# ParCoreLab/aCG

Measured on AMD Instinct MI355X. Metric: CG iter/s (whole node), Queen_4147-shaped fp64, higher is better.
Workload: dtype fp64; 1 GPU; model=queen4147-like-27pt-dof3-G111, rows=4102893, solver=cg-classic, parallelism=slab1-rccl

## Files before the change

acg_amd/gen/device_slab.py:

```python

from __future__ import annotations

import numpy as np
import torch

from ..part.subdomain import HaloPattern
from .stencil import _blocks, _slab_bounds


class DeviceSlabSystem:

    def __init__(self, **kw):
        self.__dict__.update(kw)

    @property
    def nlocal(self):
        return self.nowned + self.nghost

    @property
    def nnzA(self):
        return self._nnzA

    @property
    def nnzO(self):
        return self._nnzO


def estimate_slab_gib(gx: int, gy: int, gz: int, spec: dict, rank: int,
                      nranks: int, matfree: bool = False) -> float:
    dof = spec["dof"]
# ... 189 lines not shown
        sendidx_parts.append(plane_rows(z1 - 1))
    sendcounts = [len(s) for s in sendidx_parts]
    sdispls = list(np.concatenate([[0], np.cumsum(sendcounts)[:-1]])) if sendcounts else []
    sendidx = (np.concatenate(sendidx_parts) if sendidx_parts
               else np.zeros(0, np.int64))
    halo = HaloPattern(
        senders=np.asarray(senders, dtype=np.int32),
        recvcounts=np.asarray(recvcounts, dtype=np.int64),
        rdispls=np.asarray(rdispls, dtype=np.int64),
        recipients=np.asarray(recipients, dtype=np.int32),
        sendcounts=np.asarray(sendcounts, dtype=np.int64),
        sdispls=np.asarray(sdispls, dtype=np.int64),
        sendidx=sendidx.astype(np.int32),
    )
    return DeviceSlabSystem(
        rank=rank, nparts=nranks, n_global=gx * gy * gz * dof,
        nowned=nowned, ninterior=ninterior_nodes * dof,
        nborder=nborder_nodes * dof, nghost=nghost,
        A_sell=(A_sellptr, A_cols, A_vals) if operator else None,
        A_bsell=A_bsell,
        O_sell=(O_sellptr, O_cols, O_vals) if operator else None,
        mf_tables=mf_tables,
        _nnzA=nnzA, _nnzO=nnzO, halo=halo, device=device,
    )
```

acg_amd/gen/stencil.py:

```python

from __future__ import annotations

import numpy as np

from ..core.symcsr import SymCSRMatrix
from ..part.subdomain import HaloPattern, LocalSystem

def _offsets_27():
    offs = [(dx, dy, dz, -1.0)
            for dz in (-1, 0, 1) for dy in (-1, 0, 1) for dx in (-1, 0, 1)
            if not (dx == 0 and dy == 0 and dz == 0)]
    return offs


STENCIL_5PT_2D = {
    "offsets": [(-1, 0, 0, -1.0), (1, 0, 0, -1.0), (0, -1, 0, -1.0), (0, 1, 0, -1.0)],
    "diag": 4.0,
    "dof": 1,
}
STENCIL_7PT_3D = {
    "offsets": [(-1, 0, 0, -1.0), (1, 0, 0, -1.0), (0, -1, 0, -1.0),
                (0, 1, 0, -1.0), (0, 0, -1, -1.0), (0, 0, 1, -1.0)],
    "diag": 6.0,
    "dof": 1,
# ... 55 lines not shown
            ii.append(gid * dof + a)
            jj.append(gid * dof + b)
            vv.append(np.full(nnodes, D[a, b]))
    for (dx, dy, dz, w) in spec["offsets"]:
        if (dz, dy, dx) <= (0, 0, 0):
            continue
        nx, ny, nz = X + dx, Y + dy, Z + dz
        ok = (nx >= 0) & (nx < gx) & (ny >= 0) & (ny < gy) & (nz >= 0) & (nz < gz)
        gi = gid[ok]
        gj = _node_id(nx[ok], ny[ok], nz[ok], gx, gy)
        for a in range(dof):
            for b in range(dof):
                if M[a, b] == 0.0:
                    continue
                ii.append(gi * dof + a)
                jj.append(gj * dof + b)
                vv.append(np.full(len(gi), w * M[a, b]))
    i = np.concatenate(ii)
    j = np.concatenate(jj)
    v = np.concatenate(vv)
    return SymCSRMatrix.from_coo(n, i, j, v)


def _slab_bounds(gz: int, rank: int, nranks: int) -> tuple[int, int]:
    z0 = (gz * rank) // nranks
    z1 = (gz * (rank + 1)) // nranks
    return z0, z1


def stencil_local_slab(gx: int, gy: int, gz: int, spec: dict,
                       rank: int, nranks: int) -> LocalSystem:
    dof = spec["dof"]
    z0, z1 = _slab_bounds(gz, rank, nranks)
    nz_own = z1 - z0
    if nz_own <= 0:
        raise ValueError(f"rank {rank} has no z-planes ({gz} planes / {nranks} ranks)")
    plane_nodes = gx * gy
    has_lo = rank > 0
    has_hi = rank < nranks - 1
    maxreach = max(abs(o[2]) for o in spec["offsets"])
    if maxreach > 1:
        raise ValueError("slab generator supports |dz| <= 1 stencils")
    border_planes = set()
    if has_lo:
        border_planes.add(z0)
    if has_hi:
# ... 122 lines not shown
        recipients.append(rank + 1)
        sendidx_parts.append(plane_rows(z1 - 1))
    if has_lo and has_hi:
        pass
    sendcounts = [len(s) for s in sendidx_parts]
    sdispls = list(np.concatenate([[0], np.cumsum(sendcounts)[:-1]])) if sendcounts else []
    sendidx = np.concatenate(sendidx_parts) if sendidx_parts else np.zeros(0, np.int64)

    halo = HaloPattern(
        senders=np.asarray(senders, dtype=np.int32),
        recvcounts=np.asarray(recvcounts, dtype=np.int64),
        rdispls=np.asarray(rdispls, dtype=np.int64),
        recipients=np.asarray(recipients, dtype=np.int32),
        sendcounts=np.asarray(sendcounts, dtype=np.int64),
        sdispls=np.asarray(sdispls, dtype=np.int64),
        sendidx=sendidx.astype(cdt),
    )
    return LocalSystem(
        rank=rank, nparts=nranks, n_global=gx * gy * gz * dof,
        nowned=nowned, ninterior=ninterior, nborder=nborder, nghost=nghost,
        A_rowptr=A_rowptr, A_colidx=A_cols.astype(cdt), A_vals=A_vals,
        O_rowptr=O_rowptr, O_colidx=O_cols.astype(cdt), O_vals=O_vals,
        owned_global=owned_global, ghost_global=ghost_global, halo=halo,
    )
```

acg_amd/ops/gpu_ops.py:

```python

from __future__ import annotations

import torch

try:
    from . import _acg_kernels as K
except ImportError as e:
    raise ImportError(
        "acg_amd HIP kernel extension (_acg_kernels) is not built. "
        "Run `python -m acg_amd.ops.build` (hipcc --offload-arch=gfx950). "
        f"Original error: {e}"
    ) from e

S_RR = K.S_RR
S_PT = K.S_PT
S_RR_PREV = K.S_RR_PREV
S_BNRM2 = K.S_BNRM2
S_GAMMA = K.S_GAMMA
S_DELTA = K.S_DELTA
S_GAMMA_PREV = K.S_GAMMA_PREV
S_ALPHA_PREV = K.S_ALPHA_PREV
S_NSLOTS = K.S_NSLOTS
MAXG = K.MAXG


def _stream() -> int:
    return torch.cuda.current_stream().cuda_stream


def alloc_scalars(device) -> torch.Tensor:
    return torch.zeros(S_NSLOTS, dtype=torch.float64, device=device)


def alloc_partials(device) -> torch.Tensor:
    return torch.zeros(2 * MAXG, dtype=torch.float64, device=device)


def pick_lanes(mean_nnz_per_row: float) -> int:
    if mean_nnz_per_row <= 4.0:
        return 4
    if mean_nnz_per_row <= 8.0:
        return 8
    if mean_nnz_per_row <= 16.0:
        return 16
    if mean_nnz_per_row <= 96.0:
        return 32
# ... 119 lines not shown
                1 if cols.dtype == torch.int64 else 0,
                vals.data_ptr(), x.data_ptr(), y.data_ptr(), accum,
                partials.data_ptr() if fuse else 0,
                scal.data_ptr() if fuse else 0, dotslot, dot_accum,
                variant, perm.data_ptr() if perm is not None else 0, val32,
                _stream())


def spmv_bsell(bptr: torch.Tensor, bcol: torch.Tensor, bvals: torch.Tensor,
               nnodes: int, dof: int, x: torch.Tensor, y: torch.Tensor, *,
               partials: torch.Tensor | None = None,
               scal: torch.Tensor | None = None, dotslot: int = -1,
               dot_accum: bool = True) -> None:
    val32 = _val32(bvals, "spmv_bsell")
    nslices = bptr.numel() - 1
    if nslices <= 0:
        return
    fuse = scal is not None and dotslot >= 0
    K.spmv_bsell(nslices, nnodes, dof, bptr.data_ptr(), bcol.data_ptr(),
                 bvals.data_ptr(), x.data_ptr(), y.data_ptr(),
                 partials.data_ptr() if fuse else 0,
                 scal.data_ptr() if fuse else 0, dotslot, dot_accum, val32,
                 _stream())


def stencil_spmv(mf, nrows_nodes: int, row0_node: int, x: torch.Tensor,
                 y: torch.Tensor, *, mato: bool = False,
                 partials: torch.Tensor | None = None,
                 scal: torch.Tensor | None = None, dotslot: int = -1,
                 dot_accum: bool = True) -> None:
    if nrows_nodes <= 0:
        return
    fuse = scal is not None and dotslot >= 0
    pp = partials.data_ptr() if fuse else 0
    sp = scal.data_ptr() if fuse else 0
    if not mato and mf["w7"] is not None:
        K.stencil_spmv7(mf["gx"] * mf["gy"], mf["gx"], mf["z0"], mf["z1"],
                        mf["gz"], mf["nown_nodes"], mf["pb"].data_ptr(),
                        mf["diag"], *mf["w7"], x.data_ptr(), y.data_ptr(),
                        pp, sp, dotslot, dot_accum, _stream())
        return
    K.stencil_spmv(nrows_nodes, row0_node, mf["gx"], mf["gy"], mf["gz"],
                   mf["nown_nodes"], mf["zs"].data_ptr(),
                   mf["pb"].data_ptr(), mf["offs"].data_ptr(), mf["ksten"],
                   mf["diag"], x.data_ptr(), y.data_ptr(), mato,
                   pp, sp, dotslot, dot_accum, _stream())
# ... 526 lines not shown
```

acg_amd/ops/kernels.hip:

```cpp
#define S_RR 0
#define S_PT 1
#define S_RR_PREV 2
#define S_BNRM2 3
#define S_GAMMA 4
#define S_DELTA 5
#define S_GAMMA_PREV 6
#define S_ALPHA_PREV 7
#define S_NSLOTS 8

#define BS_LD 8
#define BS_M 0
#define BS_XI 64
#define BS_XIC 128
#define BS_G 192
#define BS_ZETA 256
#define BS_ZINV 320
#define BS_C 384
#define BS_FLAG 448
#define BS_ITER 449
#define BS_SIZE 456
#define BLOCK_MAXG 2048
#define BLOCK_TAU 1e-6

#define MAXG 16384
// ... 185 lines not shown
        double acc[DOF];
        #pragma unroll
        for (int r = 0; r < DOF; ++r) acc[r] = 0.0;
        for (long j = 0; j < blen; ++j) {
            const int cb = ld_nt(c + j * WAVE);
            double xv[DOF];
            #pragma unroll
            for (int cc = 0; cc < DOF; ++cc) xv[cc] = x[(long)cb * DOF + cc];
            const ValT* __restrict__ vj = v + j * (DOF * DOF) * WAVE;
            #pragma unroll
            for (int k = 0; k < DOF * DOF; ++k) {
                const double a = (double)ld_nt(vj + bval_off<DOF * DOF>(k, lane));
                acc[k / DOF] += a * xv[k % DOF];
            }
        }
        const long node = s * WAVE + lane;
        if (node < nnodes) {
            #pragma unroll
            for (int r = 0; r < DOF; ++r) {
                y[node * DOF + r] = acc[r];
                if (FUSE_DOT) dacc += x[node * DOF + r] * acc[r];
            }
        }
    }
    if (FUSE_DOT) {
        dacc = block_reduce(dacc);
        if (threadIdx.x == 0) partials[blockIdx.x] = dacc;
    }
}

template <int DOF>
__global__ void __launch_bounds__(BLOCK)
k_spmv_bsell_daypx(long nslices, long nnodes,
                   const long* __restrict__ bptr,
                   const int* __restrict__ bcol,
                   const double* __restrict__ bvals,
                   const double* __restrict__ pold,
                   const double* __restrict__ rvec,
                   double* __restrict__ pnew,
                   double* __restrict__ y,
                   const double* __restrict__ scal,
                   double* __restrict__ partials) {
    const int lane = threadIdx.x & (WAVE - 1);
    const long wslice = ((long)blockIdx.x * BLOCK + threadIdx.x) >> 6;
    const long nw = ((long)gridDim.x * BLOCK) >> 6;
    const double beta = safe_div(scal[S_RR], scal[S_RR_PREV]);
// ... 692 lines not shown
                               (int)blocks, (double*)scal, dotslot, dot_accum ? 1 : 0);
            check_hip("spmv_bsell_reduce");
        }
        return;
    }
    #define LBS(D, FD) \
        hipLaunchKernelGGL((k_spmv_bsell<D, FD>), g, b, 0, (hipStream_t)stream, \
            nslices, nnodes, (const long*)bptr, (const int*)bcol, \
            (const double*)bvals, (const double*)x, (double*)y, (double*)partials)
    switch (dof) {
        case 2: if (fuse) { LBS(2, true); } else { LBS(2, false); } break;
        case 3: if (fuse) { LBS(3, true); } else { LBS(3, false); } break;
        case 4: if (fuse) { LBS(4, true); } else { LBS(4, false); } break;
        default: throw std::runtime_error("spmv_bsell: dof must be 2/3/4");
    }
    #undef LBS
    check_hip("spmv_bsell");
    if (fuse) {
        hipLaunchKernelGGL(k_reduce_partials, dim3(1), dim3(BLOCK), 0,
                           (hipStream_t)stream, (const double*)partials,
                           (int)blocks, (double*)scal, dotslot, dot_accum ? 1 : 0);
        check_hip("spmv_bsell_reduce");
    }
}

void spmv_bsell_daypx(long nslices, long nnodes, int dof, uintptr_t bptr,
                      uintptr_t bcol, uintptr_t bvals, uintptr_t pold,
                      uintptr_t rvec, uintptr_t pnew, uintptr_t y,
                      uintptr_t scal, uintptr_t partials, int dotslot,
                      uintptr_t stream) {
    if (nnodes == 0) return;
    long blocks = (nslices * WAVE + BLOCK - 1) / BLOCK;
    if (blocks > MAXG) blocks = MAXG;
    dim3 g((unsigned)blocks), b(BLOCK);
    #define LBD(D) \
        hipLaunchKernelGGL((k_spmv_bsell_daypx<D>), g, b, 0, (hipStream_t)stream, \
            nslices, nnodes, (const long*)bptr, (const int*)bcol, \
            (const double*)bvals, (const double*)pold, (const double*)rvec, \
            (double*)pnew, (double*)y, (const double*)scal, (double*)partials)
    switch (dof) {
        case 2: LBD(2); break;
        case 3: LBD(3); break;
        case 4: LBD(4); break;
        default: throw std::runtime_error("spmv_bsell_daypx: dof must be 2/3/4");
    }
    #undef LBD
// ... 1891 lines not shown
    m.def("spmv_sell", &spmv_sell);
    m.def("zero_scalars", &zero_scalars);
    m.def("cg_prep_pt", &cg_prep_pt);
    m.def("cg_prep_rr", &cg_prep_rr);
    m.def("dot", &dot);
    m.def("dot2", &dot2);
    m.def("axpy_ratio", &axpy_ratio);
    m.def("daypx_ratio", &daypx_ratio);
    m.def("cg_fused_update", &cg_fused_update);
    m.def("pcg_fused_update", &pcg_fused_update);
    m.def("bsell_diag_inv", &bsell_diag_inv);
    m.def("bjacobi_apply", &bjacobi_apply);
    m.def("bpcg_fused_update", &bpcg_fused_update);
    m.def("pipelined_fused", &pipelined_fused);
    m.def("sell_pipe", &sell_pipe);
    m.def("pipelined_finalize", &pipelined_finalize);
    m.def("pack_gather", &pack_gather);
    m.def("atomic_probe", &atomic_probe);
    m.def("cg_device", &cg_device);
    m.def("stencil_rowlen", &stencil_rowlen);
    m.def("stencil_fill", &stencil_fill);
    m.def("spmv_bsell", &spmv_bsell);
    m.def("spmv_bsell_daypx", &spmv_bsell_daypx);
    m.def("stencil_blocklen", &stencil_blocklen);
    m.def("stencil_bfill", &stencil_bfill);
    m.def("stencil_spmv", &stencil_spmv);
    m.def("stencil_pipe", &stencil_pipe);
    m.def("stencil_spmv7", &stencil_spmv7);
    m.def("stencil_pipe7", &stencil_pipe7);
    m.attr("S_RR") = S_RR;
    m.attr("S_PT") = S_PT;
    m.attr("S_RR_PREV") = S_RR_PREV;
    m.attr("S_BNRM2") = S_BNRM2;
    m.attr("S_GAMMA") = S_GAMMA;
    m.attr("S_DELTA") = S_DELTA;
    m.attr("S_GAMMA_PREV") = S_GAMMA_PREV;
    m.attr("S_ALPHA_PREV") = S_ALPHA_PREV;
    m.attr("S_NSLOTS") = S_NSLOTS;
    m.attr("MAXG") = MAXG;
}
```

acg_amd/ops/torch_ref.py:

```python

from __future__ import annotations

import math

import torch

S_RR, S_PT, S_RR_PREV, S_BNRM2 = 0, 1, 2, 3
S_GAMMA, S_DELTA, S_GAMMA_PREV, S_ALPHA_PREV = 4, 5, 6, 7
S_NSLOTS = 8
MAXG = 16384
OPERATOR_VALUE_DTYPES = (torch.float64, torch.float32)


def _vals64(vals, what: str):
    if vals.dtype not in OPERATOR_VALUE_DTYPES:
        raise TypeError(f"{what}: operator values must be float64 or "
                        f"float32, got {vals.dtype}")
    return vals.to(torch.float64)


def alloc_scalars(device="cpu") -> torch.Tensor:
    return torch.zeros(S_NSLOTS, dtype=torch.float64, device=device)


# ... 272 lines not shown
    if bptr.numel() - 1 <= 0:
        return
    n = nnodes * dof
    contrib = _bsell_contrib(bptr, bcol, bvals, nnodes, dof, x)
    y[:n] = contrib
    if scal is not None and dotslot >= 0:
        d = torch.dot(x[:n], contrib)
        scal[dotslot] = scal[dotslot] + d if dot_accum else d


def spmv_bsell_daypx(bptr, bcol, bvals, nnodes: int, dof: int, pold, rvec,
                     pnew, y, scal, partials, dotslot: int) -> None:
    if bptr.numel() - 1 <= 0:
        return
    n = nnodes * dof
    beta = _sdiv(float(scal[S_RR]), float(scal[S_RR_PREV]))
    pn = beta * pold[:n] + rvec[:n]
    contrib = _bsell_contrib(bptr, bcol, bvals, nnodes, dof, pn)
    pnew[:n] = pn
    y[:n] = contrib
    scal[dotslot] = torch.dot(pn, contrib)


def cg_prep_pt(scal) -> None:
    scal[S_PT] = 0.0


def cg_prep_rr(scal) -> None:
    scal[S_RR_PREV] = scal[S_RR].clone()


def dot(x, y, partials, scal, slot, n=None, accumulate=False) -> None:
    n = x.numel() if n is None else n
    d = torch.dot(x[:n], y[:n])
    scal[slot] = scal[slot] + d if accumulate else d


def dot2(r, w, partials, scal, n, accumulate=False) -> None:
    g = torch.dot(r[:n], r[:n])
    d = torch.dot(w[:n], r[:n])
    if accumulate:
        scal[S_GAMMA] += g
        scal[S_DELTA] += d
    else:
        scal[S_GAMMA] = g
        scal[S_DELTA] = d
# ... 616 lines not shown
```

acg_amd/part/subdomain.py:

```python

from __future__ import annotations

from dataclasses import dataclass, field

import numpy as np

from ..utils.errors import AcgError, ErrCode


@dataclass
class HaloPattern:

    senders: np.ndarray = field(default_factory=lambda: np.zeros(0, np.int32))
    recvcounts: np.ndarray = field(default_factory=lambda: np.zeros(0, np.int64))
    rdispls: np.ndarray = field(default_factory=lambda: np.zeros(0, np.int64))
    recipients: np.ndarray = field(default_factory=lambda: np.zeros(0, np.int32))
    sendcounts: np.ndarray = field(default_factory=lambda: np.zeros(0, np.int64))
    sdispls: np.ndarray = field(default_factory=lambda: np.zeros(0, np.int64))
    sendidx: np.ndarray = field(default_factory=lambda: np.zeros(0, np.int64))

    @property
    def nsenders(self) -> int:
        return len(self.senders)

# ... 9 lines not shown
    def recvsize(self) -> int:
        return int(self.recvcounts.sum()) if len(self.recvcounts) else 0


@dataclass
class LocalSystem:

    rank: int
    nparts: int
    n_global: int
    nowned: int
    ninterior: int
    nborder: int
    nghost: int
    A_rowptr: np.ndarray
    A_colidx: np.ndarray
    A_vals: np.ndarray
    O_rowptr: np.ndarray
    O_colidx: np.ndarray
    O_vals: np.ndarray
    owned_global: np.ndarray
    ghost_global: np.ndarray
    halo: HaloPattern

    @property
    def nlocal(self) -> int:
        return self.nowned + self.nghost

    @property
    def nnzA(self) -> int:
        return int(self.A_rowptr[-1])

    @property
    def nnzO(self) -> int:
        return int(self.O_rowptr[-1]) if len(self.O_rowptr) else 0

    def dump(self, file=None) -> None:
        import sys

        f = file or sys.stderr
        h = self.halo
        print(f"LocalSystem(rank={self.rank}/{self.nparts}, n_global={self.n_global})",
              file=f)
        print(f"  rows: owned={self.nowned} (interior={self.ninterior}, "
              f"border={self.nborder}), ghost={self.nghost}", file=f)
        print(f"  matA: nnz={self.nnzA}; matO: nnz={self.nnzO}", file=f)
# ... 148 lines not shown
```

acg_amd/solvers/hip.py:

```python

from __future__ import annotations

import math
import os
import sys
import time

import numpy as np
import torch

from ..dist.halo import HaloExchange
from ..ops import gpu_ops as ops
from ..part.subdomain import LocalSystem
from .base import (ColumnTolerances, SolveResult, block_results,
                   cg_flops_per_iter, check_multi_shapes, next_multi_k,
                   refine, solve_multi_by_column)


class LaggedReadback:

    def __init__(self, width: int, lag: int):
        self.lag = lag
        self._buf = [torch.zeros(width, dtype=torch.float64, pin_memory=True)
                     for _ in range(lag + 1)]
        self._ev = [torch.cuda.Event() for _ in range(lag + 1)]

    def push(self, k: int, src: torch.Tensor, stream) -> None:
        j = k % (self.lag + 1)
        if stream == torch.cuda.current_stream(stream.device):
            self._buf[j].copy_(src, non_blocking=True)
        else:
            with torch.cuda.stream(stream):
                self._buf[j].copy_(src, non_blocking=True)
        self._ev[j].record(stream)

    def event(self, k: int):
        return self._ev[k % (self.lag + 1)]

    def get(self, j: int) -> torch.Tensor:
# ... 11 lines not shown
                 profile: bool = False, matfree: bool = False,
                 force_format: str | None = None):
        self.local = local
        self.comm = comm
        if device is None:
            device = comm.device if comm is not None and comm.device is not None \
                else torch.device("cuda", 0)
        self.device = torch.device(device)
        L = local

        def up(a, dtype=None):
            t = torch.from_numpy(np.ascontiguousarray(a))
            return t.to(self.device, non_blocking=True)

        self.n = L.nowned
        self.nlocal = L.nowned + L.nghost
        self.sell = None
        self.sellO = None
        self.sell_perm = None
        self.A_rowptr = self.A_colidx = self.A_vals = None
        self.O_rowptr = self.O_colidx = self.O_vals = None
        self.lanesA = self.lanesO = lanes or 16
        self.bsell = None
        self.hybrid = None
        self.matfree = None
        if matfree:
            mf = getattr(L, "mf_tables", None)
            if mf is None:
                raise ValueError(
                    "matfree=True needs a device-generated dof=1 stencil "
                    "system (gen.device_slab with spec dof==1)")
            self.matfree = mf
        if hasattr(L, "A_sell"):
            self.sell = L.A_sell
            self.sellO = L.O_sell
            self.bsell = getattr(L, "A_bsell", None)
            if self.sell is None and self.matfree is None:
                raise ValueError("system generated with operator=False "
                                 "requires matfree=True")
        else:
            self.A_rowptr = up(L.A_rowptr)
            self.A_colidx = up(L.A_colidx)
            self.A_vals = up(L.A_vals)
            self.O_rowptr = up(L.O_rowptr)
            self.O_colidx = up(L.O_colidx)
            self.O_vals = up(L.O_vals)
            mean_nnz = L.nnzA / max(L.nowned, 1)
            self.lanesA = lanes or ops.pick_lanes(mean_nnz)
            mean_nnzO = L.nnzO / max(L.nborder, 1)
            self.lanesO = lanes or ops.pick_lanes(mean_nnzO)
            self._pick_format(L, up, use_sell, force_format)
        self.can_megafuse = (
            self.matfree is not None
            or (self.sell is not None and self.sell_perm is None
                and self.sell[1].dtype == torch.int32
                and (L.nnzO == 0 or (self.sellO is not None
                                     and self.sellO[1].dtype == torch.int32))))
        self.megafuse_auto = (self.can_megafuse
                              and (self.matfree is not None
                                   or L.nnzA / max(L.nowned, 1) <= 16.0))
        self.halo = HaloExchange(L.halo, L.nowned, self.device, comm)
        self.scal = ops.alloc_scalars(self.device)
        self.partials = ops.alloc_partials(self.device)
        from .profiling import EventProfiler

        self.prof = EventProfiler(profile)
        self.comm_stream = torch.cuda.Stream(self.device)
        self.allred_stream = torch.cuda.Stream(self.device)
        self.copy_stream = torch.cuda.Stream(self.device)
        self._rr_host = torch.zeros(1, dtype=torch.float64, pin_memory=True)
        self._ev_p = torch.cuda.Event()
        self._ev_recv = torch.cuda.Event()
        self._ev_rr = torch.cuda.Event()
        self.niterations_total = 0
        self._ws: dict = {}
        self._graphs: dict = {}
        self._nstag = 0
        self._vals32 = None
        self.multi_group = 8

    def _pick_format(self, L, up, use_sell: bool, force: str | None) -> None:
        from ..ops.torch_ref import bsell_from_csr, sell_from_csr

# ... 45 lines not shown
        def mk_bsell():
            for dof_try in (4, 3, 2):
                out = bsell_from_csr(L.A_rowptr, L.A_colidx, L.A_vals, dof_try)
                if out is None:
                    continue
                bptr_h, bcol_h, bvals_h, density = out
                if density >= 0.75:
                    self.bsell = (up(bptr_h), up(bcol_h), up(bvals_h), dof_try)
                    return True
            return False

        if force == "csr":
            return
        if force == "hybrid":
            mk_hybrid()
            return
        if force == "binned":
            mk_binned()
            return
        if force == "sell":
            mk_sell(1)
        elif force == "sigma":
            mk_sell(4096)
        elif force == "bsell":
            if not mk_bsell():
                raise ValueError("force_format=bsell: no dense dof x dof "
                                 "block structure (density < 0.75)")
        elif use_sell:
            waste = mk_sell(1)
            if waste > 0.3:
                self.sell = self.sellO = self.sell_perm = None
                waste = mk_sell(16)
                if waste > 0.5:
                    self.sell = self.sellO = self.sell_perm = None
                    mk_hybrid()
            mk_bsell()
        if self.sell is not None or self.bsell is not None:
            self.A_rowptr = self.A_colidx = self.A_vals = None

    def _workspace(self, key: str, names) -> dict:
        ws = self._ws.setdefault(key, {})
        for nm, nghost in names:
            if nm not in ws:
                n = self.nlocal if nghost else self.n
                off = 520 * self._nstag
                self._nstag += 1
                buf = torch.zeros(n + off, dtype=torch.float64,
                                  device=self.device)
                ws[nm] = buf[off:] if off else buf
        return ws


    def _allreduce_slot(self, slot: int, count: int = 1):
        if self.comm is not None and self.comm.size > 1:
            self.comm.allreduce_(self.scal[slot:slot + count])

    def _halo_fork(self, x: torch.Tensor, span=None) -> None:
        self._ev_p.record(torch.cuda.current_stream(self.device))
        self.comm_stream.wait_event(self._ev_p)
        if span is not None:
            span.__enter__()
# ... 40 lines not shown
        from .profiling import annotate_op_stats

        idxb = None
        if self.matfree is not None:
            idxb = -8.0
        elif self.bsell is not None:
            idxb = 4.0 / (self.bsell[3] ** 2)
        annotate_op_stats(res, self.local, self.prof.collect(),
                          idx_bytes_per_nnz=idxb)
        self.prof.reset()

    def _format_name(self) -> str:
        if self.matfree is not None:
            return "matrix-free"
        if hasattr(self.local, "A_sell"):
            return "device-generated"
        if self.bsell is not None:
            return "bsell"
        if self.sell is not None:
            return "sigma" if self.sell_perm is not None else "sell"
        if self.hybrid is not None:
            return "hybrid" if self.hybrid["sellptr"] is not None else "binned"
        return "csr"

    def _lowprec_values(self) -> torch.Tensor:
        if self._vals32 is None and self.n == 0:
            self._vals32 = torch.empty(0, dtype=torch.float32,
                                       device=self.device)
        if self._vals32 is None:
            fmt = self._format_name()
            if fmt not in ("sell", "sigma", "bsell"):
                raise ValueError(
                    f"the fp32-stored operator needs the SELL, sigma-SELL or "
                    f"BSELL format; this system uses {fmt}")
            src = self.bsell[2] if self.bsell is not None else self.sell[2]
            self._vals32 = src.to(torch.float32)
        return self._vals32

    def _spmv_overlapped(self, xfull: torch.Tensor, y: torch.Tensor,
                         fuse_dotslot: int = -1, lowprec: bool = False):
        L = self.local
        vals32 = self._lowprec_values() if lowprec else None
        have_halo = self.comm is not None and self.comm.size > 1
        if have_halo:
            halo_span = self.prof.span("halo", self.comm_stream)
            self._halo_fork(xfull, halo_span)
# ... 71 lines not shown

    def solve(self, b: torch.Tensor, x: torch.Tensor, maxits: int = 100,
              res_atol: float = 0.0, res_rtol: float = 1e-9,
              use_graph: bool | None = None,
              fold_daypx: bool | None = None,
              diff_atol: float = 0.0, diff_rtol: float = 0.0) -> SolveResult:
        return self._solve_classic(b, x, maxits, res_atol, res_rtol,
                                   use_graph, fold_daypx, diff_atol,
                                   diff_rtol, lowprec=False)

    def _solve_classic(self, b, x, maxits, res_atol, res_rtol,
                       use_graph=None, fold_daypx=None, diff_atol=0.0,
                       diff_rtol=0.0, *, lowprec: bool) -> SolveResult:
        gkey = "classic:f32" if lowprec else "classic"
        res = SolveResult(solver="cg-hip", maxits=maxits, res_atol=res_atol,
                          res_rtol=res_rtol,
                          nranks=self.comm.size if self.comm else 1)
        n = self.n
        S = ops
        scal = self.scal
        ws = self._workspace("classic", [("r", False), ("t", False),
                                         ("p", True), ("xi", True)])
        r, t, p, xi = ws["r"], ws["t"], ws["p"], ws["xi"]
        xi.copy_(x)
        torch.cuda.synchronize(self.device)
        t0 = time.perf_counter()
        S.dot(b, b, self.partials, scal, S.S_BNRM2, n=n)
        self._allreduce_slot(S.S_BNRM2)
        self._spmv_overlapped(xi, t, lowprec=lowprec)
        torch.sub(b[:n], t, out=r)
        p[:n] = r
        S.dot(r, r, self.partials, scal, S.S_RR, n=n)
        self._allreduce_slot(S.S_RR)
        bnrm2sqr = self._host_scalar(S.S_BNRM2)
        rr = self._host_scalar(S.S_RR)
        res.bnrm2 = math.sqrt(max(bnrm2sqr, 0.0))
        res.r0nrm2 = math.sqrt(max(rr, 0.0))
        rtol2 = max(res_atol, res_rtol * res.bnrm2) ** 2
        dtol = max(diff_atol, diff_rtol * res.bnrm2)
        if rtol2 > 0 and rr <= rtol2 and dtol == 0.0:
            res.converged = True
            res.rnrm2 = math.sqrt(rr)
            res.tsolve = time.perf_counter() - t0
            return res
        converged = False
        serial = self.comm is None or self.comm.size == 1
        if dtol > 0:
            converged = self._solve_diffmode(res, r, t, p, xi, rtol2, dtol,
                                             maxits)
            return self._finish_classic(res, x, xi, converged, rtol2, t0)
        fold = (serial and self.bsell is not None and self.local.nnzO == 0
                and fold_daypx is True)
        if fold:
# ... 1 lines not shown
            scal[S.S_RR_PREV] = math.inf
        if use_graph is None:
            use_graph = not serial
        graph_ok = use_graph and serial and not self.prof.enabled and not fold
        graph = self._graphs.get(gkey) if graph_ok else None
        dist_key = gkey + ":dist"
        dist_failed_key = "classic:capture_failed"
        dist_graph_ok = (not fold
                         and self._dist_capture_ok(use_graph, dist_failed_key))
        dgraph = self._graphs.get(dist_key) if dist_graph_ok else None
        ring = LaggedReadback(1, lag=2)

        def body(k: int = 0):
            if fold:
                bptr, bcol, bvals, dof = self.bsell
                pold, pnew = (p, p2) if k % 2 == 0 else (p2, p)
                with self.prof.span("spmvA"):
                    S.spmv_bsell_daypx(bptr, bcol, bvals, n // dof, dof,
                                       pold, r, pnew, t, scal,
                                       self.partials, S.S_PT)
                with self.prof.span("update_classic"):
                    S.cg_fused_update(r, xi, pnew, t, scal, self.partials, n)
                return
            self._spmv_overlapped(p, t, fuse_dotslot=S.S_PT, lowprec=lowprec)
            with self.prof.span("allreduce"):
                self._allreduce_slot(S.S_PT)
            with self.prof.span("update_classic"):
                S.cg_fused_update(r, xi, p, t, scal, self.partials, n)
            with self.prof.span("allreduce"):
                self._allreduce_slot(S.S_RR)
            with self.prof.span("daypx"):
                S.daypx_ratio(p, r, scal, S.S_RR, S.S_RR_PREV, n=n)

        def check(j):
            nonlocal rr, converged
            rr = float(ring.get(j)[0])
            if not math.isfinite(rr):
                raise FloatingPointError(f"CG diverged: rr={rr} at it {j + 1}")
            if rtol2 > 0 and rr <= rtol2:
                converged = True
                res.niterations = j + 1
                return True
            return False

        k = 0
        cur = torch.cuda.current_stream(self.device)
        rr_slot = scal[S.S_RR:S.S_RR + 1]
# ... 3 lines not shown
            if graph is not None:
                graph.replay()
            elif dgraph is not None and k > 0:
                dgraph.replay()
            else:
                body(k)
                if graph_ok and k == 1:
                    graph = torch.cuda.CUDAGraph()
                    with torch.cuda.graph(graph):
                        body()
                    self._graphs[gkey] = graph
                elif dist_graph_ok and k == 2 and dgraph is None:
                    dgraph = self._capture_dist(body, dist_failed_key,
                                                "classic ")
                    if dgraph is not None:
                        self._graphs[dist_key] = dgraph
            ring.push(k, rr_slot, cur)
            k += 1
            res.niterations = k
        if not converged:
            for j in ring.tail(maxits):
                if check(j):
                    break
        return self._finish_classic(res, x, xi, converged, rtol2, t0)

    def _solve_diffmode(self, res, r, t, p, xi, rtol2: float, dtol: float,
                        maxits: int) -> bool:
        S = ops
        n = self.n
        scal = self.scal
        converged = False
        for k in range(maxits):
            self._spmv_overlapped(p, t, fuse_dotslot=S.S_PT)
            self._allreduce_slot(S.S_PT)
            S.dot(p, p, self.partials, scal, S.S_GAMMA, n=n)
            self._allreduce_slot(S.S_GAMMA)
            S.cg_fused_update(r, xi, p, t, scal, self.partials, n)
            self._allreduce_slot(S.S_RR)
            res.niterations = k + 1
            rr_old = self._host_scalar(S.S_RR_PREV)
            pt = self._host_scalar(S.S_PT)
            pp = self._host_scalar(S.S_GAMMA)
            rr = self._host_scalar(S.S_RR)
            if not math.isfinite(rr):
                raise FloatingPointError(f"CG diverged: rr={rr} at it {k + 1}")
            alpha = rr_old / pt if pt != 0.0 else 0.0
            dx = abs(alpha) * math.sqrt(max(pp, 0.0))
            if (rtol2 > 0 and rr <= rtol2) or dx <= dtol:
                converged = True
                break
            S.daypx_ratio(p, r, scal, S.S_RR, S.S_RR_PREV, n=n)
        return converged

    def _finish_classic(self, res, x, xi, converged: bool, rtol2: float,
                        t0: float):
        S = ops
        torch.cuda.synchronize(self.device)
        res.tsolve = time.perf_counter() - t0
        x.copy_(xi)
        rr = self._host_scalar(S.S_RR)
        res.rnrm2 = math.sqrt(max(rr, 0.0))
        res.converged = converged or (rtol2 > 0 and rr <= rtol2)
        nnz_full = self.local.nnzA + self.local.nnzO
        self._count_work(res, cg_flops_per_iter(nnz_full, self.n))
        self._annotate_profile(res)
        return res


    def _multi_fast_path(self) -> bool:
        serial = self.comm is None or self.comm.size == 1
        return (serial and self.matfree is None and self.local.nnzO == 0
                and self.n > 0
                and (self.bsell is not None or self.sell is not None))

    def _multi_kmax(self) -> int:
        if self.multi_group not in ops.MULTI_K:
            raise ValueError(f"multi_group must be one of {ops.MULTI_K}, "
                             f"got {self.multi_group}")
        ok = [k for k in ops.MULTI_K if k <= self.multi_group
              and (self.bsell is None
                   or ops.spmm_bsell_supported(self.bsell[3], k))]
        return max(ok) if ok else 0
# ... 747 lines not shown
```

Before: 1808 iter/s.

## Add symmetric-tile BSELL SpMV that stores each in-tile block pair once

Introduces a new operator format for serial classic CG. Nodes are renumbered in brick order, and for symmetric block pairs that land in the same 256-node tile only one copy is stored. The kernel computes the transpose product and scatters it through LDS to the receiving row, which cuts matrix value traffic from HBM. It is enabled by default and adds permutation of the inputs and outputs around the solve, extra LDS use, a synchronisation per tile, and a host-side build step that may fall back if the matrix is not exactly symmetric.

```diff
diff --git a/acg_amd/gen/device_slab.py b/acg_amd/gen/device_slab.py
--- a/acg_amd/gen/device_slab.py
+++ b/acg_amd/gen/device_slab.py
@@ -5,7 +5,7 @@
 import torch
 
 from ..part.subdomain import HaloPattern
-from .stencil import _blocks, _slab_bounds
+from .stencil import _blocks, _slab_bounds, brick_order
 
 
 class DeviceSlabSystem:
@@ -241,4 +241,5 @@
         O_sell=(O_sellptr, O_cols, O_vals) if operator else None,
         mf_tables=mf_tables,
         _nnzA=nnzA, _nnzO=nnzO, halo=halo, device=device,
+        node_order=brick_order(gx, gy, gz) if nranks == 1 else None,
     )
diff --git a/acg_amd/gen/stencil.py b/acg_amd/gen/stencil.py
--- a/acg_amd/gen/stencil.py
+++ b/acg_amd/gen/stencil.py
@@ -101,6 +101,17 @@
     return SymCSRMatrix.from_coo(n, i, j, v)
 
 
+def brick_order(gx: int, gy: int, gz: int,
+                brick: tuple[int, int, int] = (8, 8, 4)) -> np.ndarray:
+    bx, by, bz = brick
+    z, y, x = np.meshgrid(np.arange(gz), np.arange(gy), np.arange(gx),
+                          indexing="ij")
+    nbx, nby = -(-gx // bx), -(-gy // by)
+    key = ((((z // bz) * nby + y // by) * nbx + x // bx) * bz + z % bz) * by
+    key = ((key + y % by) * bx + x % bx).ravel()
+    return np.argsort(key, kind="stable").astype(np.int64)
+
+
 def _slab_bounds(gz: int, rank: int, nranks: int) -> tuple[int, int]:
     z0 = (gz * rank) // nranks
     z1 = (gz * (rank + 1)) // nranks
@@ -269,4 +280,5 @@
         A_rowptr=A_rowptr, A_colidx=A_cols.astype(cdt), A_vals=A_vals,
         O_rowptr=O_rowptr, O_colidx=O_cols.astype(cdt), O_vals=O_vals,
         owned_global=owned_global, ghost_global=ghost_global, halo=halo,
+        node_order=brick_order(gx, gy, gz) if nranks == 1 else None,
     )
diff --git a/acg_amd/ops/gpu_ops.py b/acg_amd/ops/gpu_ops.py
--- a/acg_amd/ops/gpu_ops.py
+++ b/acg_amd/ops/gpu_ops.py
@@ -22,6 +22,7 @@
 S_ALPHA_PREV = K.S_ALPHA_PREV
 S_NSLOTS = K.S_NSLOTS
 MAXG = K.MAXG
+K_ST_TILE = 256
 
 
 def _stream() -> int:
@@ -187,6 +188,29 @@
                  partials.data_ptr() if fuse else 0,
                  scal.data_ptr() if fuse else 0, dotslot, dot_accum, val32,
                  _stream())
+
+
+def spmv_bsell_st(st, x: torch.Tensor, y: torch.Tensor, *,
+                  partials: torch.Tensor | None = None,
+                  scal: torch.Tensor | None = None, dotslot: int = -1,
+                  dot_accum: bool = True, max_blocks: int = 0) -> int:
+    if st.tile != K_ST_TILE:
+        raise ValueError(f"spmv_bsell_st: the kernel's tile is {K_ST_TILE} "
+                         f"nodes, this operator was built with {st.tile}")
+    n = st.nnodes * st.dof
+    if x.numel() < n or y.numel() < n:
+        raise ValueError("spmv_bsell_st: x and y must hold nnodes * dof values")
+    if x.dtype != torch.float64 or y.dtype != torch.float64:
+        raise TypeError("spmv_bsell_st: x and y must be float64")
+    fuse = scal is not None and dotslot >= 0
+    return K.spmv_bsell_st(st.ntiles, st.nslices, st.nnodes, st.dof, st.qmax,
+                           st.sptr.data_ptr(), st.spl.data_ptr(),
+                           st.scol.data_ptr(), st.sq.data_ptr(),
+                           st.svals.data_ptr(), st.nrecv.data_ptr(),
+                           x.data_ptr(), y.data_ptr(),
+                           partials.data_ptr() if fuse else 0,
+                           scal.data_ptr() if fuse else 0, dotslot, dot_accum,
+                           max_blocks, _stream())
 
 
 def stencil_spmv(mf, nrows_nodes: int, row0_node: int, x: torch.Tensor,
diff --git a/acg_amd/ops/kernels.hip b/acg_amd/ops/kernels.hip
--- a/acg_amd/ops/kernels.hip
+++ b/acg_amd/ops/kernels.hip
@@ -231,6 +231,103 @@
                 if (FUSE_DOT) dacc += x[node * DOF + r] * acc[r];
             }
         }
+    }
+    if (FUSE_DOT) {
+        dacc = block_reduce(dacc);
+        if (threadIdx.x == 0) partials[blockIdx.x] = dacc;
+    }
+}
+
+#define ST_NOSEND 255
+
+template <int DOF, bool FUSE_DOT>
+__global__ void __launch_bounds__(BLOCK)
+k_spmv_bsell_st(long ntiles, long nslices, long nnodes,
+                const long* __restrict__ sptr,
+                const int* __restrict__ spl,
+                const int* __restrict__ scol,
+                const unsigned char* __restrict__ sq,
+                const double* __restrict__ svals,
+                const unsigned char* __restrict__ nrecv,
+                const double* __restrict__ x,
+                double* __restrict__ y,
+                double* __restrict__ partials) {
+    extern __shared__ double st_lds[];
+    const int lane = threadIdx.x & (WAVE - 1);
+    const int wid = threadIdx.x >> 6;
+    double dacc = 0.0;
+    for (long t = blockIdx.x; t < ntiles; t += gridDim.x) {
+        const long tile_base = t * BLOCK;
+        const long s = t * (BLOCK / WAVE) + wid;
+        const long node = tile_base + threadIdx.x;
+        const bool live = s < nslices;
+        double acc[DOF];
+        #pragma unroll
+        for (int r = 0; r < DOF; ++r) acc[r] = 0.0;
+        if (live) {
+            const long nself = node < nnodes ? node : nnodes - 1;
+            double xs[DOF];
+            #pragma unroll
+            for (int r = 0; r < DOF; ++r) xs[r] = x[nself * DOF + r];
+            const long b0 = sptr[s];
+            const long blen = (sptr[s + 1] - b0) >> 6;
+            const long npl = spl[s];
+            const int* __restrict__ c = scol + b0 + lane;
+            const unsigned char* __restrict__ qp = sq + b0 + lane;
+            const double* __restrict__ v = svals + b0 * (DOF * DOF);
+            #pragma unroll 2
+            for (long j = 0; j < npl; ++j) {
+                const int cb = ld_nt(c + j * WAVE);
+                double xv[DOF];
+                #pragma unroll
+                for (int cc = 0; cc < DOF; ++cc) xv[cc] = x[(long)cb * DOF + cc];
+                const double* __restrict__ vj = v + j * (DOF * DOF) * WAVE;
+                #pragma unroll
+                for (int k = 0; k < DOF * DOF; ++k) {
+                    const double a = ld_nt(vj + bval_off<DOF * DOF>(k, lane));
+                    acc[k / DOF] += a * xv[k % DOF];
+                }
+            }
+            #pragma unroll 2
+            for (long j = npl; j < blen; ++j) {
+                const int cb = ld_nt(c + j * WAVE);
+                const int q = ld_nt(qp + j * WAVE);
+                double xv[DOF], tr[DOF];
+                #pragma unroll
+                for (int cc = 0; cc < DOF; ++cc) {
+                    xv[cc] = x[(long)cb * DOF + cc];
+                    tr[cc] = 0.0;
+                }
+                const double* __restrict__ vj = v + j * (DOF * DOF) * WAVE;
+                #pragma unroll
+                for (int k = 0; k < DOF * DOF; ++k) {
+                    const double a = ld_nt(vj + bval_off<DOF * DOF>(k, lane));
+                    acc[k / DOF] += a * xv[k % DOF];
+                    tr[k % DOF] += a * xs[k / DOF];
+                }
+                if (q != ST_NOSEND) {
+                    const int loc = (int)((long)cb - tile_base);
+                    #pragma unroll
+                    for (int cc = 0; cc < DOF; ++cc)
+                        st_lds[(q * DOF + cc) * BLOCK + loc] = tr[cc];
+                }
+            }
+        }
+        __syncthreads();
+        if (live && node < nnodes) {
+            const int nr = nrecv[node];
+            for (int q = 0; q < nr; ++q) {
+                #pragma unroll
+                for (int r = 0; r < DOF; ++r)
+                    acc[r] += st_lds[(q * DOF + r) * BLOCK + threadIdx.x];
+            }
+            #pragma unroll
+            for (int r = 0; r < DOF; ++r) {
+                y[node * DOF + r] = acc[r];
+                if (FUSE_DOT) dacc += x[node * DOF + r] * acc[r];
+            }
+        }
+        __syncthreads();
     }
     if (FUSE_DOT) {
         dacc = block_reduce(dacc);
@@ -969,6 +1066,52 @@
                            (int)blocks, (double*)scal, dotslot, dot_accum ? 1 : 0);
         check_hip("spmv_bsell_reduce");
     }
+}
+
+long spmv_bsell_st(long ntiles, long nslices, long nnodes, int dof, int qmax,
+                   uintptr_t sptr, uintptr_t spl, uintptr_t scol, uintptr_t sq,
+                   uintptr_t svals, uintptr_t nrecv, uintptr_t x, uintptr_t y,
+                   uintptr_t partials, uintptr_t scal, int dotslot,
+                   bool dot_accum, long max_blocks, uintptr_t stream) {
+    if (nnodes == 0 || ntiles == 0) return 0;
+    if (ntiles != (nslices + BLOCK / WAVE - 1) / (BLOCK / WAVE)
+        || nslices != (nnodes + WAVE - 1) / WAVE)
+        throw std::invalid_argument("spmv_bsell_st: tile/slice/node counts disagree");
+    if (qmax < 0 || qmax >= ST_NOSEND)
+        throw std::invalid_argument("spmv_bsell_st: qmax must be in [0, 255)");
+    const size_t lds = (size_t)qmax * dof * BLOCK * sizeof(double);
+    if (lds > 96 * 1024)
+        throw std::invalid_argument("spmv_bsell_st: qmax * dof needs more than 96 KiB of LDS");
+    long blocks = ntiles;
+    if (blocks > MAXG) blocks = MAXG;
+    if (max_blocks > 0 && blocks > max_blocks) blocks = max_blocks;
+    const bool fuse = partials != 0 && dotslot >= 0;
+    dim3 g((unsigned)blocks), b(BLOCK);
+    #define LST(D, FD) do { \
+        if (lds > 48 * 1024 && hipFuncSetAttribute( \
+                (const void*)k_spmv_bsell_st<D, FD>, \
+                hipFuncAttributeMaxDynamicSharedMemorySize, (int)lds) != hipSuccess) \
+            throw std::runtime_error("spmv_bsell_st: cannot raise the LDS limit"); \
+        hipLaunchKernelGGL((k_spmv_bsell_st<D, FD>), g, b, lds, (hipStream_t)stream, \
+            ntiles, nslices, nnodes, (const long*)sptr, (const int*)spl, \
+            (const int*)scol, (const unsigned char*)sq, (const double*)svals, \
+            (const unsigned char*)nrecv, (const double*)x, (double*)y, \
+            (double*)partials); } while (0)
+    switch (dof) {
+        case 2: if (fuse) { LST(2, true); } else { LST(2, false); } break;
+        case 3: if (fuse) { LST(3, true); } else { LST(3, false); } break;
+        case 4: if (fuse) { LST(4, true); } else { LST(4, false); } break;
+        default: throw std::runtime_error("spmv_bsell_st: dof must be 2/3/4");
+    }
+    #undef LST
+    check_hip("spmv_bsell_st");
+    if (fuse) {
+        hipLaunchKernelGGL(k_reduce_partials, dim3(1), dim3(BLOCK), 0,
+                           (hipStream_t)stream, (const double*)partials,
+                           (int)blocks, (double*)scal, dotslot, dot_accum ? 1 : 0);
+        check_hip("spmv_bsell_st_reduce");
+    }
+    return blocks;
 }
 
 void spmv_bsell_daypx(long nslices, long nnodes, int dof, uintptr_t bptr,
@@ -2906,6 +3049,8 @@
     m.def("stencil_fill", &stencil_fill);
     m.def("spmv_bsell", &spmv_bsell);
     m.def("spmv_bsell_daypx", &spmv_bsell_daypx);
+    m.def("spmv_bsell_st", &spmv_bsell_st);
+    m.attr("ST_NOSEND") = ST_NOSEND;
     m.def("stencil_blocklen", &stencil_blocklen);
     m.def("stencil_bfill", &stencil_bfill);
     m.def("stencil_spmv", &stencil_spmv);
diff --git a/acg_amd/ops/symtile.py b/acg_amd/ops/symtile.py
--- /dev/null
+++ b/acg_amd/ops/symtile.py
@@ -0,0 +1,197 @@
+
+from __future__ import annotations
+
+from types import SimpleNamespace
+
+import torch
+
+C = 64
+TILE = 256
+QMAX = 8
+GATE = 0.9
+NOSEND = 255
+
+
+def val_index(pos: torch.Tensor, lane: torch.Tensor, d2: int) -> torch.Tensor:
+    k = torch.arange(d2, device=pos.device)[None, :]
+    even = d2 & ~1
+    lane = lane[:, None]
+    off = torch.where(k < even, (k >> 1) * (2 * C) + lane * 2 + (k & 1),
+                      even * C + lane)
+    return (pos[:, None] - lane) * d2 + off
+
+
+def stored_bytes(nblocks: int, nslot_bytes: int, nslices: int, d2: int) -> int:
+    return (nblocks * (8 * d2 + 4) + nslot_bytes + nslices * C
+            + (nslices + 1) * 8 + nslices * 4)
+
+
+def bsell_bytes(nblocks: int, nslices: int, d2: int) -> int:
+    return nblocks * (8 * d2 + 4) + (nslices + 1) * 8
+
+
+def _decode(ptr, col, vals, nnodes, d2):
+    nsl = ptr.numel() - 1
+    dev = ptr.device
+    pos = torch.arange(int(ptr[-1]), device=dev)
+    sl = torch.repeat_interleave(torch.arange(nsl, device=dev), ptr[1:] - ptr[:-1])
+    lane = (pos - ptr[sl]) % C
+    return sl * C + lane, col.long(), vals[val_index(pos, lane, d2)], pos, sl
+
+
+def bsell_st_build(bptr, bcol, bvals, nnodes: int, dof: int, node_order=None,
+                   *, tile: int = TILE, qmax: int = QMAX, gate: float = GATE):
+    if bvals.dtype != torch.float64:
+        raise TypeError(f"bsell_st_build: float64 block values, got {bvals.dtype}")
+    if not 0 <= qmax < NOSEND:
+        raise ValueError(f"bsell_st_build: qmax must be in [0, {NOSEND})")
+    if tile < 1 or (tile > C and tile % C):
+        raise ValueError("bsell_st_build: tile must be a multiple of 64 (or < 64)")
+    dev = bptr.device
+    d2 = dof * dof
+    nsl = bptr.numel() - 1
+    if nnodes <= 0 or nsl != (nnodes + C - 1) // C:
+        raise ValueError("bsell_st_build: bptr does not match nnodes")
+    ar = torch.arange(nnodes, device=dev)
+    if node_order is None:
+        order = ar
+    else:
+        order = torch.as_tensor(node_order).to(dev).long()
+        if order.shape != (nnodes,) or not torch.equal(order.sort().values, ar):
+            raise ValueError("bsell_st_build: node_order is not a permutation")
+    inv0 = torch.empty_like(order)
+    inv0[order] = ar
+
+    node, col, vals, _, _ = _decode(bptr, bcol, bvals, nnodes, d2)
+    real = (node < nnodes) & (vals != 0).any(dim=1)
+    i0, j0, vals = inv0[node[real]], inv0[col[real]], vals[real]
+    key, srt = torch.sort(i0 * nnodes + j0)
+    if key.numel() > 1 and bool((key[1:] == key[:-1]).any()):
+        return None
+    i0, j0, vals = i0[srt], j0[srt], vals[srt]
+    nb = key.numel()
+
+    e = torch.nonzero((i0 // tile == j0 // tile) & (i0 != j0)).squeeze(1)
+    if e.numel():
+        pkey = j0[e] * nnodes + i0[e]
+        pidx = torch.searchsorted(key, pkey).clamp_(max=nb - 1)
+        if not bool((key[pidx] == pkey).all()):
+            return None
+        vt = vals[e].view(-1, dof, dof).transpose(1, 2).reshape(-1, d2).contiguous()
+        if not torch.equal(vt.view(torch.int64),
+                           vals[pidx].contiguous().view(torch.int64)):
+            return None
+        low = i0[e] < j0[e]
+        blo, bhi = e[low], pidx[low]
+    else:
+        blo = bhi = e
+    a, b = i0[blo], j0[blo]
+    npairs = blo.numel()
+
+    stored = torch.bincount(i0, minlength=nnodes)
+    got = torch.zeros(nnodes, dtype=torch.int64, device=dev)
+    recv = torch.full((npairs,), -1, dtype=torch.int64, device=dev)
+    pid = torch.arange(npairs, device=dev)
+    prio = (((pid * 2654435761) & 0x7FFFFFFF) << 32) | pid
+    big = torch.iinfo(torch.int64).max
+    for _ in range(8 * qmax + 8 if npairs and qmax else 0):
+        capa, capb = got[a] >= qmax, got[b] >= qmax
+        sa, sb = stored[a], stored[b]
+        a_claims = ~capa & ((sa >= sb) | capb)
+        b_claims = ~capb & ((sb > sa) | capa)
+        who = torch.where(a_claims, a, torch.where(b_claims, b, -1))
+        cand = (recv < 0) & (who >= 0)
+        if not bool(cand.any()):
+            break
+        best = torch.full((nnodes,), big, dtype=torch.int64, device=dev)
+        best.scatter_reduce_(0, who[cand], prio[cand], "amin")
+        win = cand & (best[who.clamp(min=0)] == prio)
+        recv[win] = torch.where(who == a, 0, 1)[win]
+        w = who[win]
+        stored[w] -= 1
+        got[w] += 1
+    done = recv >= 0
+    a_recv = recv == 0
+    drop_b = torch.where(a_recv, blo, bhi)[done]
+    send_b = torch.where(a_recv, bhi, blo)[done]
+    receiver0 = torch.where(a_recv, a, b)[done]
+    owner0 = torch.where(a_recv, b, a)[done]
+
+    cmax = int(stored.max())
+    order1 = torch.sort((ar // tile) * (cmax + 1) + (cmax - stored),
+                        stable=True).indices
+    inv1 = torch.empty_like(order1)
+    inv1[order1] = ar
+    perm = order[order1]
+    iperm = torch.empty_like(perm)
+    iperm[perm] = ar
+
+    q = torch.full((nb,), NOSEND, dtype=torch.int64, device=dev)
+    nrecv = torch.zeros(nsl * C, dtype=torch.int64, device=dev)
+    if send_b.numel():
+        r1, o1 = inv1[receiver0], inv1[owner0]
+        rk, rs = torch.sort(r1 * nnodes + o1)
+        r1s = r1[rs]
+        cnt = torch.bincount(r1s, minlength=nnodes)
+        start = torch.cumsum(cnt, 0) - cnt
+        q[send_b[rs]] = torch.arange(rs.numel(), device=dev) - start[r1s]
+        nrecv[:nnodes] = cnt
+    assert int(nrecv.max()) <= qmax
+
+    keep = torch.ones(nb, dtype=torch.bool, device=dev)
+    keep[drop_b] = False
+    i1, j1, vals, q = inv1[i0[keep]], inv1[j0[keep]], vals[keep], q[keep]
+    sends = (q != NOSEND).long()
+    srt = torch.sort((i1 * 2 + sends) * nnodes + j1).indices
+    i1, j1, vals, q, sends = i1[srt], j1[srt], vals[srt], q[srt], sends[srt]
+    total = torch.bincount(i1, minlength=nnodes)
+    nplain = total - torch.bincount(i1, weights=sends.double(),
+                                    minlength=nnodes).long()
+    within = torch.arange(i1.numel(), device=dev) - (torch.cumsum(total, 0) - total)[i1]
+    pad = torch.zeros(nsl * C, dtype=torch.int64, device=dev)
+    pad[:nnodes] = total
+    blen = pad.view(nsl, C).max(dim=1).values
+    pad.fill_(big)
+    pad[:nnodes] = nplain
+    spl = torch.minimum(pad.view(nsl, C).min(dim=1).values, blen)
+    sptr = torch.zeros(nsl + 1, dtype=torch.int64, device=dev)
+    torch.cumsum(blen * C, dim=0, out=sptr[1:])
+    stotal = int(sptr[-1])
+    pos = torch.arange(stotal, device=dev)
+    sl = torch.repeat_interleave(torch.arange(nsl, device=dev), blen * C)
+    lane = (pos - sptr[sl]) % C
+    scol = torch.clamp(sl * C + lane, max=nnodes - 1).to(torch.int32)
+    sq = torch.full((stotal,), NOSEND, dtype=torch.uint8, device=dev)
+    svals = torch.zeros(stotal * d2, dtype=torch.float64, device=dev)
+    dst = sptr[i1 // C] + within * C + i1 % C
+    scol[dst] = j1.to(torch.int32)
+    sq[dst] = q.to(torch.uint8)
+    svals[val_index(dst, i1 % C, d2)] = vals
+    snd = q != NOSEND
+    assert bool((within[snd] >= spl[i1[snd] // C]).all())
+    assert bool((j1[snd] // tile == i1[snd] // tile).all())
+
+    nslot = int(((blen - spl) * C).sum())
+    sbytes = stored_bytes(stotal, nslot, nsl, d2)
+    bbytes = bsell_bytes(int(bptr[-1]), nsl, d2)
+    if sbytes > gate * bbytes:
+        return None
+    dofs = torch.arange(dof, device=dev)
+    return SimpleNamespace(
+        sptr=sptr, spl=spl.to(torch.int32), scol=scol, sq=sq, svals=svals,
+        nrecv=nrecv.to(torch.uint8), perm=perm, iperm=iperm,
+        vperm=(perm[:, None] * dof + dofs[None, :]).reshape(-1),
+        nnodes=nnodes, dof=dof, tile=tile, qmax=qmax,
+        ntiles=(nnodes + tile - 1) // tile, nslices=nsl,
+        nblocks=stotal, nslot_bytes=nslot, stored_bytes=sbytes,
+        bsell_bytes=bbytes, ratio=sbytes / bbytes,
+        npairs=int(npairs), npaired=int(send_b.numel()))
+
+
+def decode_st(st):
+    d2 = st.dof * st.dof
+    node, col, vals, pos, sl = _decode(st.sptr, st.scol, st.svals, st.nnodes, d2)
+    j = (pos - st.sptr[sl]) // C
+    q = torch.where(j >= st.spl.long()[sl], st.sq.long(),
+                    torch.full_like(j, NOSEND))
+    return node, col, vals, q
diff --git a/acg_amd/ops/torch_ref.py b/acg_amd/ops/torch_ref.py
--- a/acg_amd/ops/torch_ref.py
+++ b/acg_amd/ops/torch_ref.py
@@ -318,6 +318,33 @@
     scal[dotslot] = torch.dot(pn, contrib)
 
 
+def spmv_bsell_st(st, x, y, *, partials=None, scal=None, dotslot: int = -1,
+                  dot_accum: bool = True, max_blocks: int = 0) -> None:
+    from .symtile import NOSEND, decode_st
+
+    nn, dof = st.nnodes, st.dof
+    n = nn * dof
+    node, col, vals, q = decode_st(st)
+    live = node < nn
+    node, col, vals, q = node[live], col[live], vals[live], q[live]
+    A = vals.view(-1, dof, dof)
+    xb = x[:n].view(nn, dof)
+    contrib = torch.zeros(nn, dof, dtype=torch.float64, device=x.device)
+    contrib.index_add_(0, node, torch.einsum("brc,bc->br", A, xb[col]))
+    snd = q != NOSEND
+    slots = torch.zeros(max(st.qmax, 1), nn, dof, dtype=torch.float64,
+                        device=x.device)
+    slots[q[snd], col[snd]] = torch.einsum("brc,br->bc", A[snd], xb[node[snd]])
+    nr = st.nrecv[:nn].long()
+    for s in range(st.qmax):
+        contrib += torch.where((nr > s)[:, None], slots[s], 0.0)
+    contrib = contrib.reshape(-1)
+    y[:n] = contrib
+    if scal is not None and dotslot >= 0:
+        d = torch.dot(x[:n], contrib)
+        scal[dotslot] = scal[dotslot] + d if dot_accum else d
+
+
 def cg_prep_pt(scal) -> None:
     scal[S_PT] = 0.0
 
diff --git a/acg_amd/part/subdomain.py b/acg_amd/part/subdomain.py
--- a/acg_amd/part/subdomain.py
+++ b/acg_amd/part/subdomain.py
@@ -55,6 +55,7 @@
     owned_global: np.ndarray
     ghost_global: np.ndarray
     halo: HaloPattern
+    node_order: np.ndarray | None = None
 
     @property
     def nlocal(self) -> int:
diff --git a/acg_amd/solvers/hip.py b/acg_amd/solvers/hip.py
--- a/acg_amd/solvers/hip.py
+++ b/acg_amd/solvers/hip.py
@@ -15,6 +15,9 @@
 from .base import (ColumnTolerances, SolveResult, block_results,
                    cg_flops_per_iter, check_multi_shapes, next_multi_k,
                    refine, solve_multi_by_column)
+
+
+BSELL_ST_DEFAULT = True
 
 
 class LaggedReadback:
@@ -72,6 +75,7 @@
         self.O_rowptr = self.O_colidx = self.O_vals = None
         self.lanesA = self.lanesO = lanes or 16
         self.bsell = None
+        self.bsell_st = None
         self.hybrid = None
         self.matfree = None
         if matfree:
@@ -109,6 +113,7 @@
         self.megafuse_auto = (self.can_megafuse
                               and (self.matfree is not None
                                    or L.nnzA / max(L.nowned, 1) <= 16.0))
+        self._build_symtile(force_format)
         self.halo = HaloExchange(L.halo, L.nowned, self.device, comm)
         self.scal = ops.alloc_scalars(self.device)
         self.partials = ops.alloc_partials(self.device)
@@ -200,9 +205,9 @@
             mk_sell(1)
         elif force == "sigma":
             mk_sell(4096)
-        elif force == "bsell":
+        elif force in ("bsell", "bsell-st"):
             if not mk_bsell():
-                raise ValueError("force_format=bsell: no dense dof x dof "
+                raise ValueError(f"force_format={force}: no dense dof x dof "
                                  "block structure (density < 0.75)")
         elif use_sell:
             waste = mk_sell(1)
@@ -215,6 +220,29 @@
             mk_bsell()
         if self.sell is not None or self.bsell is not None:
             self.A_rowptr = self.A_colidx = self.A_vals = None
+
+    def _build_symtile(self, force: str | None) -> None:
+        from ..ops.symtile import bsell_st_build
+
+        env = os.environ.get("ACG_BSELL_ST", "")
+        serial = self.comm is None or self.comm.size == 1
+        wanted = force == "bsell-st" or (
+            force is None and (env == "1" or (BSELL_ST_DEFAULT and env != "0")))
+        if (wanted and env != "0" and serial and self.local.nnzO == 0
+                and self.bsell is not None and self.matfree is None):
+            bptr, bcol, bvals, dof = self.bsell
+            self.bsell_st = bsell_st_build(
+                bptr, bcol, bvals, self.n // dof, dof,
+                getattr(self.local, "node_order", None))
+            if self.bsell_st is not None:
+                print(f"# classic CG operator format: bsell-st "
+                      f"({self.bsell_st.ratio:.3f} of the bsell bytes)",
+                      file=sys.stderr, flush=True)
+        if force == "bsell-st" and self.bsell_st is None:
+            raise ValueError(
+                "force_format=bsell-st: not built (needs one rank, no matO, "
+                "ACG_BSELL_ST != 0, exact transposes inside every tile and "
+                "stored bytes <= 0.9 of BSELL's)")
 
     def _workspace(self, key: str, names) -> dict:
         ws = self._ws.setdefault(key, {})
@@ -301,6 +329,10 @@
         if self.hybrid is not None:
             return "hybrid" if self.hybrid["sellptr"] is not None else "binned"
         return "csr"
+
+    @property
+    def classic_format(self) -> str:
+        return "bsell-st" if self.bsell_st is not None else self._format_name()
 
     def _lowprec_values(self) -> torch.Tensor:
         if self._vals32 is None and self.n == 0:
@@ -418,13 +450,34 @@
         ws = self._workspace("classic", [("r", False), ("t", False),
                                          ("p", True), ("xi", True)])
         r, t, p, xi = ws["r"], ws["t"], ws["p"], ws["xi"]
-        xi.copy_(x)
+        st = self.bsell_st
+        if lowprec or fold_daypx is True or diff_atol > 0 or diff_rtol > 0:
+            st = None
+
+        def spmv(xv, yv, fuse_dotslot=-1):
+            if st is None:
+                self._spmv_overlapped(xv, yv, fuse_dotslot=fuse_dotslot,
+                                      lowprec=lowprec)
+                return
+            with self.prof.span("spmvA"):
+                S.spmv_bsell_st(st, xv, yv, partials=self.partials,
+                                scal=scal if fuse_dotslot >= 0 else None,
+                                dotslot=fuse_dotslot, dot_accum=False)
+
+        if st is None:
+            xi.copy_(x)
+        else:
+            torch.index_select(x[:n], 0, st.vperm, out=xi[:n])
         torch.cuda.synchronize(self.device)
         t0 = time.perf_counter()
         S.dot(b, b, self.partials, scal, S.S_BNRM2, n=n)
         self._allreduce_slot(S.S_BNRM2)
-        self._spmv_overlapped(xi, t, lowprec=lowprec)
-        torch.sub(b[:n], t, out=r)
+        spmv(xi, t)
+        if st is None:
+            torch.sub(b[:n], t, out=r)
+        else:
+            torch.index_select(b[:n], 0, st.vperm, out=r)
+            r.sub_(t)
         p[:n] = r
         S.dot(r, r, self.partials, scal, S.S_RR, n=n)
         self._allreduce_slot(S.S_RR)
@@ -472,7 +525,7 @@
                 with self.prof.span("update_classic"):
                     S.cg_fused_update(r, xi, pnew, t, scal, self.partials, n)
                 return
-            self._spmv_overlapped(p, t, fuse_dotslot=S.S_PT, lowprec=lowprec)
+            spmv(p, t, fuse_dotslot=S.S_PT)
             with self.prof.span("allreduce"):
                 self._allreduce_slot(S.S_PT)
             with self.prof.span("update_classic"):
@@ -522,7 +575,7 @@
             for j in ring.tail(maxits):
                 if check(j):
                     break
-        return self._finish_classic(res, x, xi, converged, rtol2, t0)
+        return self._finish_classic(res, x, xi, converged, rtol2, t0, st)
 
     def _solve_diffmode(self, res, r, t, p, xi, rtol2: float, dtol: float,
                         maxits: int) -> bool:
@@ -553,11 +606,14 @@
         return converged
 
     def _finish_classic(self, res, x, xi, converged: bool, rtol2: float,
-                        t0: float):
+                        t0: float, st=None):
         S = ops
         torch.cuda.synchronize(self.device)
         res.tsolve = time.perf_counter() - t0
-        x.copy_(xi)
+        if st is None:
+            x.copy_(xi)
+        else:
+            x[:self.n].index_copy_(0, st.vperm, xi[:self.n])
         rr = self._host_scalar(S.S_RR)
         res.rnrm2 = math.sqrt(max(rr, 0.0))
         res.converged = converged or (rtol2 > 0 and rr <= rtol2)
```

Measured after the change: 2046 iter/s, median of 6. +13.2%, better.
